# zhouxian/act3d-chained-diffuser

Measured on AMD Instinct MI355X. Metric: train samples/sec (Act3D keypose fwd+bwd+AdamW step), higher is better.
Workload: dtype fp16 / bf16 MFMA on two-part operands (x = hi + lo; fp32 accumulate) in attention; fp32-accurate linears (f32 MFMA; bf16x3 MFMA from 4096 rows); bf16 frozen backbone + FPN; 1 GPU; Act3D keypose training step, 18-PerAct-task shapes: 4 cameras 256x256, 3 ghost-point levels, 1000 ghost points (333/level), E=60, frozen synthetic CLIP-RN50-shaped backbone + trainable FPN included in the step; per_gpu_batch_keyframes=64, global_batch=64, parallelism=dp1, hipgraph=True, backbone_prefetch=True

## Files before the change

### act3d-chained-diffuser_amd/csrc/conv1x1_deep.hip

```cpp
#include "a3d_common.h"
#include "../../include/act3d_hip.h"

namespace a3d {

constexpr int CD_BM = 128, CD_BN = 128, CD_BK = 64;

__device__ __forceinline__ int cd_xoff(int row, int seg) { return row * 64 + ((seg ^ ((row >> 1) & 7)) << 3); }
__device__ __forceinline__ int cd_woff(int row, int seg) { return row * 64 + ((seg ^ ((((row >> 4) & 3) << 1) | ((row >> 1) & 1))) << 3); }

__device__ __forceinline__ unsigned int cd_norm2(unsigned int u, const float* scS, int K, int k, float relu_lo) {
  float a = __uint_as_float(u << 16) * scS[k] + scS[K + k];
  float b = __uint_as_float(u & 0xFFFF0000u) * scS[k + 1] + scS[K + k + 1];
  return pk_bf16(fmaxf(a, relu_lo), fmaxf(b, relu_lo));
}

__device__ __forceinline__ void cd_compute(const unsigned short* Xb, const unsigned short* Wb, const int (&xo)[2][4], const int (&wo)[2][4],
                                           f32x4 (&acc)[4][4]) {
#pragma unroll
  for (int h = 0; h < 2; ++h) {
    s16x8 xa[4], wb[4];
#pragma unroll
    for (int i = 0; i < 4; ++i) {
      xa[i] = *reinterpret_cast<const s16x8*>(&Xb[xo[h][i]]);
      wb[i] = *reinterpret_cast<const s16x8*>(&Wb[wo[h][i]]);
// ... 3 lines not shown
#pragma unroll
      for (int tm = 0; tm < 4; ++tm) acc[tn][tm] = mfma_bf16_16x16x32(wb[tn], xa[tm], acc[tn][tm]);
  }
}

__device__ __forceinline__ void cd_epilogue(f32x4 (&acc)[4][4], float (&ssum)[4][4], float (&ssq)[4][4], unsigned short* __restrict__ y,
                                            long long m0, long long M, int N, int n0, int wm, int wn, int li, int g) {
#pragma unroll
  for (int tm = 0; tm < 4; ++tm) {
    const long long m = m0 + wm * 64 + tm * 16 + li;
    const bool ok = m < M;
    unsigned int pk[8];
#pragma unroll
    for (int tn = 0; tn < 4; ++tn) {
#pragma unroll
      for (int r2 = 0; r2 < 2; ++r2) {
        const unsigned int u = pk_bf16(acc[tn][tm][2 * r2], acc[tn][tm][2 * r2 + 1]);
        const float v0 = ok ? __uint_as_float(u << 16) : 0.f, v1 = ok ? __uint_as_float(u & 0xFFFF0000u) : 0.f;
        ssum[tn][2 * r2] += v0;
        ssq[tn][2 * r2] += v0 * v0;
        ssum[tn][2 * r2 + 1] += v1;
        ssq[tn][2 * r2 + 1] += v1 * v1;
        pk[2 * tn + r2] = u;
      }
      acc[tn][tm] = f32x4{0.f, 0.f, 0.f, 0.f};
    }
    if (ok) {
      uint4* dst = reinterpret_cast<uint4*>(y + (size_t)m * N + n0 + wn * 64 + g * 16);
      dst[0] = make_uint4(pk[0], pk[1], pk[2], pk[3]);
      dst[1] = make_uint4(pk[4], pk[5], pk[6], pk[7]);
    }
  }
}

template <bool XFORM>
__global__ __launch_bounds__(256, 2) void conv1x1_deep_kernel(const unsigned short* __restrict__ x, const unsigned short* __restrict__ w,
                                                            const float* __restrict__ in_scale, const float* __restrict__ in_shift,
                                                            int in_relu, unsigned short* __restrict__ y, float* __restrict__ partial,
                                                            long long M, int N, int K) {
  extern __shared__ __attribute__((aligned(16))) unsigned short smem_cd[];
  unsigned short* Xs = smem_cd;
  unsigned short* Ws = Xs + 2 * CD_BM * CD_BK;
  float* scS = reinterpret_cast<float*>(Ws + 2 * CD_BN * CD_BK);
  const int t = threadIdx.x, lane = t & 63, wave = t >> 6;
  const int li = lane & 15, g = lane >> 4;
  const int wm = wave >> 1, wn = wave & 1;
  const int n0 = blockIdx.y * CD_BN;
  const int KS = K / CD_BK;
  const long long mtiles = (M + CD_BM - 1) / CD_BM;
  if (XFORM)
    for (int i = t; i < K; i += 256) { scS[i] = in_scale[i]; scS[K + i] = in_shift[i]; }
  float ssum[4][4], ssq[4][4];
#pragma unroll
  for (int a = 0; a < 4; ++a)
#pragma unroll
    for (int r = 0; r < 4; ++r) { ssum[a][r] = 0.f; ssq[a][r] = 0.f; }
  const long long my_tiles = blockIdx.x < mtiles ? (mtiles - blockIdx.x + gridDim.x - 1) / gridDim.x : 0;
  const long long total = my_tiles * KS;
  const int srow = t >> 3, sseg = t & 7;
  long long l_m0 = (long long)blockIdx.x * CD_BM;
  int l_ks = 0;
  const float relu_lo = in_relu ? 0.f : -INFINITY;
#define CD_LOAD1(P, i)                                                                                                \
  {                                                                                                                   \
    const long long m_ = l_m0 + srow + 32 * i < M ? l_m0 + srow + 32 * i : M - 1;    \
    P##x##i = *reinterpret_cast<const uint4*>(x + (size_t)m_ * K + l_ks * CD_BK + sseg * 8);                          \
    P##w##i = *reinterpret_cast<const uint4*>(w + (size_t)(n0 + srow + 32 * i) * K + l_ks * CD_BK + sseg * 8);        \
  }
#define CD_LOAD(P)                                                                                                    \
  do {                                                                                                                \
    CD_LOAD1(P, 0) CD_LOAD1(P, 1) CD_LOAD1(P, 2) CD_LOAD1(P, 3)                                                       \
    if (l_left > 1) { --l_left; if (++l_ks == KS) { l_ks = 0; l_m0 += (long long)gridDim.x * CD_BM; } }               \
  } while (0)
#define CD_STAGE1(P, i)                                                                                               \
  {                                                                                                                   \
    uint4 v = P##x##i;                                                                                                \
    if (XFORM) {                                                                                                      \
      const int k0 = ks * CD_BK + sseg * 8;                                                                           \
      unsigned int u0 = v.x, u1 = v.y, u2 = v.z, u3 = v.w;                                                            \
      u0 = cd_norm2(u0, scS, K, k0 + 0, relu_lo); u1 = cd_norm2(u1, scS, K, k0 + 2, relu_lo);                         \
      u2 = cd_norm2(u2, scS, K, k0 + 4, relu_lo); u3 = cd_norm2(u3, scS, K, k0 + 6, relu_lo);                         \
      v = make_uint4(u0, u1, u2, u3);                                                                                 \
    }                                                                                                                 \
    *reinterpret_cast<uint4*>(&Xs[buf * CD_BM * CD_BK + cd_xoff(srow + 32 * i, sseg)]) = v;                           \
    *reinterpret_cast<uint4*>(&Ws[buf * CD_BN * CD_BK + cd_woff(srow + 32 * i, sseg)]) = P##w##i;                     \
  }
#define CD_STAGE(P) CD_STAGE1(P, 0) CD_STAGE1(P, 1) CD_STAGE1(P, 2) CD_STAGE1(P, 3)
  int xo[2][4], wo[2][4];
#pragma unroll
  for (int h = 0; h < 2; ++h)
#pragma unroll
    for (int i = 0; i < 4; ++i) {
      xo[h][i] = cd_xoff(wm * 64 + i * 16 + li, h * 4 + g);
      wo[h][i] = cd_woff(wn * 64 + (li >> 2) * 16 + i * 4 + (li & 3), h * 4 + g);
    }
  if (total > 0) {
    uint4 ax0, ax1, ax2, ax3, aw0, aw1, aw2, aw3, bx0, bx1, bx2, bx3, bw0, bw1, bw2, bw3;
    long long l_left = total;
    CD_LOAD(a);
    CD_LOAD(b);
    long long c_m0 = (long long)blockIdx.x * CD_BM;
    int ks = 0;
    f32x4 acc[4][4];
#pragma unroll
    for (int a = 0; a < 4; ++a)
#pragma unroll
      for (int b = 0; b < 4; ++b) acc[a][b] = f32x4{0.f, 0.f, 0.f, 0.f};
    __syncthreads();
#define CD_STEP(P, BUF)                                                                                               \
    {                                                                                                                 \
      constexpr int buf = BUF;                                                                                        \
      CD_STAGE(P)                                                                                                     \
      CD_LOAD(P);                                                                                \
      __syncthreads();                                             \
      cd_compute(Xs + buf * CD_BM * CD_BK, Ws + buf * CD_BN * CD_BK, xo, wo, acc);                                    \
      if (ks == KS - 1) cd_epilogue(acc, ssum, ssq, y, c_m0, M, N, n0, wm, wn, li, g);                                \
      if (++ks == KS) { ks = 0; c_m0 += (long long)gridDim.x * CD_BM; }                                               \
    }
    for (long long s = 0; s < total; s += 2) {
      CD_STEP(a, 0)
      if (s + 1 < total) CD_STEP(b, 1)
    }
#undef CD_STEP
  }
  if (!partial) return;
  __syncthreads();
  float* redS = reinterpret_cast<float*>(Xs);
  float* redQ = redS + 4 * 64;
#pragma unroll
  for (int tn = 0; tn < 4; ++tn)
#pragma unroll
    for (int r = 0; r < 4; ++r) {
      float sv = ssum[tn][r], q = ssq[tn][r];
#pragma unroll
      for (int o = 1; o < 16; o <<= 1) { sv += __shfl_xor(sv, o, 64); q += __shfl_xor(q, o, 64); }
      if (li == 0) { redS[wave * 64 + g * 16 + tn * 4 + r] = sv; redQ[wave * 64 + g * 16 + tn * 4 + r] = q; }
    }
  __syncthreads();
  if (t < CD_BN) {
    const int wn_i = t >> 6, c = t & 63;
    const float sv = redS[(0 * 2 + wn_i) * 64 + c] + redS[(1 * 2 + wn_i) * 64 + c];
    const float q = redQ[(0 * 2 + wn_i) * 64 + c] + redQ[(1 * 2 + wn_i) * 64 + c];
    float* p = partial + (size_t)blockIdx.x * 2 * N;
    p[n0 + t] = sv;
    p[N + n0 + t] = q;
  }
}

#undef CD_LOAD
#undef CD_LOAD1
#undef CD_STAGE1
#undef CD_STAGE

}

using namespace a3d;

bool a3d::conv1x1_deep_serves(int K, int N) { return K >= 128 && K <= 2048 && (K % CD_BK) == 0 && N >= 128 && N <= 2048 && (N % CD_BN) == 0; }
static size_t cd_lds(int K, bool xform) { return (size_t)2 * (CD_BM + CD_BN) * CD_BK * 2 + (xform ? (size_t)2 * K * sizeof(float) : 0); }

int a3d::conv1x1_deep_slabs(size_t M, int K, int N) {
  (void)K;
  const size_t mtiles = (M + CD_BM - 1) / CD_BM;
  const int nblocks = N / CD_BN;
  return (int)std::min<size_t>(mtiles, (size_t)std::max(1, 512 / nblocks));
}

int a3d::conv1x1_deep_launch(const void* x, const void* w, const float* in_scale, const float* in_shift, int in_relu, void* y, float* partial,
                             size_t M, int K, int N, hipStream_t s) {
  if (in_scale && K > 1024) { set_error("a3d_conv1x1_bn_fwd: the folded BatchNorm-apply of the deep-layer kernel serves K <= 1024 (K=%d)", K); return A3D_ERR_ARG; }
  static bool once = false;
  if (!once) {
    (void)hipFuncSetAttribute((const void*)conv1x1_deep_kernel<false>, hipFuncAttributeMaxDynamicSharedMemorySize, 80 * 1024);
    (void)hipFuncSetAttribute((const void*)conv1x1_deep_kernel<true>, hipFuncAttributeMaxDynamicSharedMemorySize, 80 * 1024);
    once = true;
  }
  const dim3 grid(conv1x1_deep_slabs(M, K, N), N / CD_BN);
  if (in_scale)
    hipLaunchKernelGGL(conv1x1_deep_kernel<true>, grid, dim3(256), cd_lds(K, true), s, (const unsigned short*)x, (const unsigned short*)w,
                       in_scale, in_shift, in_relu, (unsigned short*)y, partial, (long long)M, N, K);
  else
    hipLaunchKernelGGL(conv1x1_deep_kernel<false>, grid, dim3(256), cd_lds(K, false), s, (const unsigned short*)x, (const unsigned short*)w,
                       in_scale, in_shift, in_relu, (unsigned short*)y, partial, (long long)M, N, K);
  return check_launch("a3d_conv1x1_bn_fwd(deep)");
}
```

### act3d-chained-diffuser_amd/lib.py

```python
import ctypes as C
import os

import torch

_PKG_DIR = os.path.dirname(os.path.abspath(__file__))
LIB_PATH = os.path.join(_PKG_DIR, os.path.basename(os.environ.get("A3D_LIB", "libact3d_hip.so")))

_p = C.c_void_p
_i = C.c_int
_f = C.c_float
_d = C.c_double
_z = C.c_size_t
_u64 = C.c_ulonglong



def _struct(name, fields):
    return type(name, (C.Structure,), {"_fields_": [(f, t) for f, t in fields]})


DnHeadParams = _struct("DnHeadParams", [(n, _p) for n in ("enc_w0", "enc_b0", "enc_w1", "enc_b1", "sem", "lang_kv")] +
                       [("S_lang", _i)] + [(n, _p) for n in ("q_w", "q_b", "out_w", "out_b", "ln_g", "ln_b")])
DnCrossParams = _struct("DnCrossParams", [(n, _p) for n in ("sem", "mod", "q_w", "q_b", "freq", "Kf", "Vt")])
DnRestParams = _struct("DnRestParams", [(n, _p) for n in (
    "c_out_w", "c_out_b", "c_ln_g", "c_ln_b", "sem", "s_mod", "s_in_w", "s_in_b", "s_out_w", "s_out_b", "s_ln_g", "s_ln_b", "freq",
    "kmask", "f_mod", "f_w1", "f_b1", "f_w2", "f_b2", "f_ln_g", "f_ln_b")] + [("F", _i)])
DnLayerParams = _struct("DnLayerParams", [("cross", DnCrossParams), ("rest", DnRestParams)])
DnTailParams = _struct("DnTailParams", [(n, _p) for n in (
    "pos_w0", "pos_b0", "pos_w1", "pos_b1", "rot_w0", "rot_b0", "rot_w1", "rot_b1", "noise", "cond_data", "cond_mask", "coef_pos",
    "coef_rot")])

QsParams = _struct("QsParams", [(n, _p) for n in ("wv", "bv", "wo", "bo", "g1", "b1", "w1", "c1", "w2", "c2", "g2", "b2")])
GradReduceRec = _struct("GradReduceRec", [("partial", _p), ("dst", _p), ("bias", _p)] +
                        [(n, _i) for n in ("nsplit", "slab_stride", "count", "row_len", "dst_stride", "group_len")])
QsGrads = _struct("QsGrads", [(n, _p) for n in ("dwv", "dbv", "dwo", "dbo", "dg1", "db1", "dw1", "dc1", "dw2", "dc2", "dg2", "db2")])

SIGNATURES = {
    "a3d_version": (_i, []),
    "a3d_last_error_string": (C.c_char_p, []),
    "a3d_linear_fwd": (_i, [_p, _i, _p, _i, _p, _p, _i, _p, _i, _i, _i, _i, _i, _i, _p]),
    "a3d_linear_wgrad": (_i, [_p, _i, _p, _i, _p, _i, _p, _i, _i, _i, _p]),
    "a3d_linear_wgrad_ws": (_i, [_p, _i, _p, _i, _p, _i, _p, _i, _i, _i, _p, _z, _p]),
    "a3d_linear_wgrad_ws_bytes": (_z, [_i, _i, _i, _i]),
    "a3d_add_layernorm_fwd": (_i, [_p, _p, _p, _p, _p, _p, _p, _i, _i, _f, _p]),
    "a3d_add_layernorm_bwd": (_i, [_p, _p, _p, _p, _p, _p, _p, _p, _p, _i, _i, _p]),
    "a3d_linear_wgrad_partials": (_i, [_p, _i, _p, _i, _i, _i, _i, _i, _p, _z, _p, _p]),
    "a3d_add_layernorm_bwd_partials_count": (_i, [_i, _i]),
    "a3d_add_layernorm_bwd_partials": (_i, [_p, _p, _p, _p, _p, _p, _p, _p, _i, _i, _p]),
    "a3d_colsum_rows_partials": (_i, [_p, _i, _i, _i, _i, _i, _p, _p]),
    "a3d_grad_reduce_table_plan": (_i, [_p, _i, _p]),
    "a3d_grad_reduce_table_upload": (_i, [_p, _p, _i, _p]),
    "a3d_grad_reduce_table": (_i, [_p, _i, _i, _p]),
    "a3d_rope_split_qk": (_i, [_p, _i, _p, _p, _f, _p, _i, _i, _i, _i, _i, _p]),
    "a3d_split_vt": (_i, [_p, _i, _p, _i, _i, _i, _i, _i, _p]),
    "a3d_proj_rope_split": (_i, [_p, _i, _p, _i, _p, _i, _p, _f, _p, _i, _p, _p, _f, _p, _i, _p, _p, _i, _i, _i, _i, _i, _p]),
    "a3d_rope_split": (_i, [_p, _i, _p, _p, _f, _p, _i, _p, _i, _i, _i, _i, _i, _p]),
    "a3d_rope_merge_bwd": (_i, [_p, _i, _p, _p, _f, _p, _i, _i, _i, _i, _i, _i, _p]),
    "a3d_attn_fwd": (_i, [_p, _p, _p, _p, _p, _p, _p, _i, _i, _i, _i, _i, _i, _i, _p]),
    "a3d_attn_fwd_ws_floats": (_z, [_i, _i, _i, _i]),
    "a3d_attn_bwd_bf16": (_i, [_p] * 15 + [_i] * 7 + [_p]),
    "a3d_rope_split16": (_i, [_p, _i, _p, _p, _f, _p, _p, _i, _i, _i, _i, _i, _i, _p]),
    "a3d_proj_rope_split16": (_i, [_p, _i, _p, _i, _p, _i, _p, _f, _p, _p, _i, _p, _f, _p, _p, _i, _p, _i, _i, _i, _i, _i, _p]),
    "a3d_ctx_kv_proj16_splits": (_i, [_i, _i]),
    "a3d_ctx_kv_proj16": (_i, [_p, _i, _p, _p, _p, _p, _p, _p, _p, _p, _p, _i, _p, _i, _i, _i, _i, _i, _i, _i, _p]),
    "a3d_attn16_fwd": (_i, [_p] * 7 + [_i] * 7 + [_p, C.c_uint, _f, _p]),
    "a3d_attn16_fwd_rows": (_i, [_p] * 7 + [_i] * 7 + [_p, C.c_uint, _f, _i, _p]),
    "a3d_conv3x3_tile_count": (_z, [_z, _i, _i]),
    "a3d_conv3x3_dgrad_tiles_ws_ints": (_z, [_z, _i, _i]),
    "a3d_conv3x3_mark_tiles": (_i, [_p, _i, _i, _i, _i, _i, _p, _p]),
    "a3d_conv3x3_dgrad_tiles": (_i, [_p, _p, _p, _p, _p, _z, _i, _i, _p]),
    "a3d_conv3x3_wgrad_tokens_ws_floats": (_z, []),
    "a3d_conv3x3_wgrad_tokens": (_i, [_p, _p, _p, _i, _i, _p, _p, _i, _i, _i, _i, _i, _i, _p]),
    "a3d_attn16_bwd_pack_bytes": (_z, [_i, _i, _i]),
    "a3d_dbg_dn_prof": (_i, [_p]),
    "a3d_attn8_operand_bytes": (_z, [_i, _i, _i]),
    "a3d_attn8_fwd": (_i, [_p] * 8 + [_i] * 7 + [_p]),
    "a3d_attn16_bwd": (_i, [_p] * 16 + [_i] * 7 + [_p, C.c_uint, _f, _p]),
    "a3d_pose_to_signal": (_i, [_p, _p, _p, _i, _i, _p]),
    "a3d_signal_to_pose": (_i, [_p, _p, _p, _i, _i, _p]),
    "a3d_traj_condition": (_i, [_p, _i, _p, _i, _p] + [_p] * 8 + [_i] * 5 + [_p]),
    "a3d_traj_rank": (_i, [_p, _p, _p, _i, _p] + [_f] * 6 + [_p] * 5 + [_i] * 4 + [_p]),
    "a3d_traj_rank_extra": (_i, [_p, _p, _p, _i, _p] + [_f] * 6 + [_p] * 5 + [_i] * 4 + [_p, _f, _p]),
    "a3d_traj_clearance_ws_floats": (_z, [_i] * 5),
    "a3d_traj_clearance": (_i, [_p, _p, _p, _p, _i, _i, _f, _i, _i, _p, _p, _p] + [_i] * 5 + [_p]),
    "a3d_traj_guide_ws_floats": (_z, [_i] * 5),
    "a3d_traj_guide": (_i, [_p, _i, _p, _p, _p, _p, _p, _i, _i, _f, _i, _i, _f, _f, _p, _p] + [_i] * 4 + [_p]),
    "a3d_traj_errors": (_i, [_p, _p, _p, _i, _i, _i, _p]),
    "a3d_keypose_errors": (_i, [_p, _p, _p, _p, _i, _p, _i, _i, _i, _p]),
    "a3d_sym_quat_loss": (_i, [_p, _p, _i, _f, _p, _p, _i, _p]),
    "a3d_sq_fwd_ws_floats": (_z, [_i, _i, _i, _i]),
    "a3d_sq_attn_fwd": (_i, [_p, _p, _p, _i, _p, _p, _i, _p, _p, _p, _p, _p, _p, _p, _i, _i, _i, _i, _i, _p]),
    "a3d_sq_bwd_ws_floats": (_z, [_i, _i, _i, _i]),
    "a3d_sq_attn_bwd": (_i, [_p, _p, _p, _i, _p, _p, _i, _p, _p, _p, _p, _p, _p, _p, _p, _p, _i, _p, _p, _i, _p, _i, _i, _i, _i,
                             _i, _p]),
    "a3d_sq_attn_bwd_acc": (_i, [_p, _p, _p, _i, _p, _p, _i, _p, _p, _p, _p, _p, _p, _p, _p, _p, _i, _p, _p, _i, _p, _i, _i, _i, _i,
                                 _i, _i, _p]),
    "a3d_qs_pre_fwd": (_i, [_p, _p, _p, _p, _p, _f, _p, _i, _i, _i, _p]),
    "a3d_qs_pre_bwd": (_i, [_p, _i, _p, _p, _f, _p, _p, _p, _p, _p, _i, _i, _i, _p]),
    "a3d_qs_save_floats": (_z, [_i, _i]),
    "a3d_qs_post_fwd": (_i, [_p, _p, _p, _p, _p, _i, _i, _i, _p]),
    "a3d_qs_post_bwd": (_i, [_p, _p, _p, _p, _p, _p, _p, _p, _p, _i, _i, _i, _p]),
    "a3d_sq_wgrad_reduce": (_i, [_p, _i, _p, _i, _p, _i, _p]),
    "a3d_dn_head": (_i, [_p, _i, _p, _p, _i, _i, _i, _i, _p]),
    "a3d_dn_cross_ws_floats": (_z, [_i, _i, _i]),
    "a3d_dn_cross": (_i, [_p, _p, _i, _p, _p, _i, _i, _i, _i, _i, _i, _i, _p]),
    "a3d_dn_rest": (_i, [_p, _p, _i, _p, _p, _p, _i, _i, _i, _i, _i, _p]),
    "a3d_dn_tail": (_i, [_p, _p, _p, _i, _p, _p, _i, _i, _i, _i, _p]),
    "a3d_dn_tail_sched": (_i, [_p, _p, _p, _i, _p, _p, _i, _i, _i, _i, _i, _p]),
    "a3d_dn_persist_splits": (_i, [_i, _i]),
    "a3d_dn_persist_sync_ints": (_z, [_i, _i, _i, _i]),
    "a3d_dn_persist_kvx_floats": (_z, [_i, _i, _i]),
    "a3d_dn_persist_prof": (_i, [_p, _i, _i, _i, _i, _p]),
    "a3d_dn_persist_xbuf_floats": (_z, [_i, _i]),
    "a3d_dn_persist": (_i, [_p, _i, _i, _i, _p, _p, _p, _p, _p, _p, _p, _p] + [_i] * 10 + [_p]),
    "a3d_dn_persist_sched": (_i, [_p, _i, _i, _i, _p, _p, _p, _p, _p, _p, _p, _p] + [_i] * 12 + [_p]),
    "a3d_dn_persist_group_of": (_i, [_i, _i, _i, _i, _p]),
    "a3d_dn_persist_group": (_i, [_p, _i, _i, _i, _p, _p, _p, _p, _p, _p, _p, _p] + [_i] * 13 + [_p]),
    "a3d_rope_rows_f32": (_i, [_p, _i, _p, _p, _f, _p, _i, _i, _i, _i, _i, _p]),
    "a3d_dropout": (_i, [_p, _p, _z, _p, C.c_uint, _f, _p]),
    "a3d_dropout_mask": (_i, [_p, _z, _p, C.c_uint, C.c_uint, C.c_uint, _f, _p]),
    "a3d_linear_fwd_drop": (_i, [_p, _i, _p, _i, _p, _p, _i, _p, _i, _i, _i, _i, _i, _i, _p, C.c_uint, _f, _p]),
    "a3d_add_layernorm_bwd_drop": (_i, [_p] * 10 + [_i, _i, _p, C.c_uint, _f, _p]),
    "a3d_attn_fwd_dropout": (_i, [_p, _p, _p, _p, _p, _p, _p, _i, _i, _i, _i, _i, _i, _i, _p, C.c_uint, _f, _p]),
    "a3d_attn_bwd_bf16_dropout": (_i, [_p] * 15 + [_i] * 7 + [_p, C.c_uint, _f, _p]),
    "a3d_pcd_downsample": (_i, [_p, _p, _i, _i, _i, _i, _i, _p]),
    "a3d_knn_topk_ws_bytes": (_z, [_i, _i]),
    "a3d_knn_topk": (_i, [_p, _p, _p, _p, _p, _i, _i, _i, _p]),
    "a3d_traj_nn_topk": (_i, [_p, _i, _p, _p, _p, _p, _i, _i, _i, _p]),
    "a3d_build_context": (_i, [_p, _p, _p, _p, _i, _i, _i, _i, _i, _p]),
    "a3d_build_context_bwd": (_i, [_p, _p, _p, _p, _i, _i, _i, _i, _i, _i, _p]),
    "a3d_build_context_bf16": (_i, [_p, _i, _p, _p, _p, _p, _i, _i, _i, _i, _i, _p]),
    "a3d_colsum_rows_ws_floats": (_z, [_i, _i, _i]),
    "a3d_colsum_rows": (_i, [_p, _i, _i, _i, _i, _i, _p, _i, _p, _p]),
    "a3d_build_context_bwd_bf16": (_i, [_p, _p, _p, _i, _p, _i, _i, _i, _i, _i, _i, _p]),
    "a3d_mask_logits_fwd": (_i, [_p, _p, _p, _i, _i, _i, _p]),
    "a3d_mask_logits_bwd": (_i, [_p, _p, _p, _p, _p, _i, _i, _i, _i, _p]),
    "a3d_argmax_gather": (_i, [_p, _p, _p, _p, _i, _i, _p]),
    "a3d_soft_ce_loss": (_i, [_p, _p, _p, _p, _p, _p, _i, _i, _f, _f, _f, _p]),
    "a3d_elem_loss": (_i, [_p, _p, _i, _i, _f, _p, _p, _p]),
    "a3d_scale_by_scalar": (_i, [_p, _p, _p, _z, _p]),
    "a3d_quat_sigmoid_fwd": (_i, [_p, _p, _p, _i, _p]),
    "a3d_quat_sigmoid_bwd": (_i, [_p, _p, _p, _p, _i, _p]),
    "a3d_ortho6d_sigmoid_fwd": (_i, [_p, _p, _p, _i, _p]),
    "a3d_ortho6d_sigmoid_bwd": (_i, [_p, _p, _p, _p, _i, _p]),
    "a3d_select_row_fwd": (_i, [_p, _p, _p, _i, _i, _i, _p]),
    "a3d_select_row_bwd": (_i, [_p, _p, _p, _i, _i, _i, _p]),
    "a3d_sample_ghost_points": (_i, [_p, _p, _p, _f, _p, _i, _i, _i, _i, _p]),
    "a3d_rng_advance": (_i, [_p, _u64, _p]),
    "a3d_philox4x32_10_host": (None, [_p, _p, _p]),
    "a3d_sincos_host": (None, [_p, _p, _p, _z]),
    "a3d_adamw_step": (_i, [_p, _p, _p, _p, _p, _p, _p, _i, _z, _z, _f, _f, _f, _f, _f, _f, _f, _p]),
    "a3d_adamw_ema_step": (_i, [_p] * 9 + [_i, _z, _z] + [_f] * 9 + [_p]),
    "a3d_adamw_clip_step": (_i, [_p] * 11 + [_i, _z, _z] + [_f] * 10 + [_p]),
    "a3d_adamw_sched_step": (_i, [_p] * 12 + [_i, _z, _z, _i] + [_d] * 3 + [_f] * 9 + [_p]),
    "a3d_swap_f32": (_i, [_p, _p, _z, _p]),
    "a3d_dbg_mfma_bf16": (_i, [_p, _p, _p, _p]),
    "a3d_dbg_mfma_f32": (_i, [_p, _p, _p, _p]),
    "a3d_dbg_cvt_pk_bf16": (_i, [_p, _p, _i, _p]),
    "a3d_bn_nslab": (_i, [_z, _i]),
    "a3d_bn_grid_cap": (_i, [_i]),
    "a3d_conv1x1_streams": (_i, [_i, _i]),
    "a3d_conv1x1_nslab": (_i, [_z, _i, _i]),
    "a3d_conv1x1_bn_fwd": (_i, [_p, _p, _p, _p, _i, _p, _p, _z, _i, _i, _p]),
    "a3d_conv1x1_topdown_serves": (_i, [_i, _i]),
    "a3d_conv1x1_topdown_fwd": (_i, [_p, _p, _p, _i, _p, _p, _z, _i, _i, _i, _i, _p]),
    "a3d_conv1x1_bn_residual_serves": (_i, [_i, _i]),
    "a3d_conv1x1_bn_residual_fwd": (_i, [_p, _p, _p, _p, _i, _p, _p, _p, _p, _p, _i, _i, _p, _z, _i, _i, _p]),
    "a3d_bn_gram_nslab": (_i, [_z, _i]),
    "a3d_bn_gram": (_i, [_p, _p, _p, _i, _p, _p, _z, _i, _i, _p]),
    "a3d_bn_gram_stats": (_i, [_p, _p, _i, _p, _i, _i, _p, _p, _p]),
    "a3d_conv3x3_serves": (_i, [_i, _i, _i, _i]),
    "a3d_conv1x1_deep_mode": (_i, [_i]),
    "a3d_stem_conv_nslab": (_i, [_z, _i, _i]),
    "a3d_stem_conv_bn_fwd": (_i, [_p, _p, _p, _p, _p, _p, _z, _i, _i, _p]),
    "a3d_conv3x3_nslab": (_i, [_z, _i, _i, _i, _i]),
    "a3d_conv3x3_bn_fwd": (_i, [_p, _p, _p, _p, _i, _p, _p, _z, _i, _i, _i, _i, _p]),
    "a3d_bn_stats": (_i, [_p, _p, _z, _i, _i, _p]),
    "a3d_bn_finalize": (_i, [_p, _i, _z, _i, _f, _f, _p, _p, _p, _p, _p, _p, _i, _p]),
    "a3d_bn_apply": (_i, [_p, _p, _p, _p, _p, _p, _p, _z, _i, _i, _p]),
    "a3d_bn_apply_pool2": (_i, [_p, _p, _p, _p, _p, _p, _i, _i, _i, _i, _i, _p]),
    "a3d_rgb_normalize_nhwc_bf16": (_i, [_p, _p, _p, _p, _z, _i, _i, _p]),
    "a3d_upsample2_add_fwd": (_i, [_p, _p, _p, _i, _p, _i, _i, _i, _i, _p]),
    "a3d_upsample2_add_bwd_ws_floats": (_z, [_i, _i, _i, _i]),
    "a3d_upsample2_add_bwd": (_i, [_p, _p, _p, _i, _p, _i, _i, _i, _i, _p]),
    "a3d_ddpm_add_noise": (_i, [_p, _p, _p, _p, _p, _p, _i, _i, _i, _i, _p]),
    "a3d_ddpm_step": (_i, [_p, _p, _p, _p, _p, _p, _p, _p, _i, _i, _i, _i, _p]),
    "a3d_ddpm_step_sched": (_i, [_p, _p, _p, _p, _p, _p, _p, _p, _i, _i, _i, _i, _i, _p]),
    "a3d_adaln_fwd": (_i, [_p, _p, _p, _i, _i, _i, _p]),
    "a3d_adaln_bwd": (_i, [_p, _p, _p, _p, _p, _i, _i, _i, _p]),
    "a3d_sinusoidal_emb": (_i, [_p, _p, _i, _i, _p]),
    "a3d_silu_fwd": (_i, [_p, _p, _z, _p]),
    "a3d_silu_bwd": (_i, [_p, _p, _p, _z, _p]),
    "a3d_add_rows": (_i, [_p, _p, _p, _i, _i, _i, _p]),
    "a3d_add_rows_bwd": (_i, [_p, _p, _i, _i, _i, _p]),
    "a3d_resize_crop": (_i, [_p, _p, _p, _i, _i, _i, _i, _f, _f, _p]),
    "a3d_traj_update": (_i, [_p, _p, _p, _i, _i, _i, _p]),
}

ADAMW_CLIP_WS_DOUBLES = 256
LR_DECAY_KINDS = {"constant": 0, "linear": 1, "cosine": 2}

_lib = None


def load():
    global _lib
    if _lib is not None:
        return _lib
    if not os.path.exists(LIB_PATH):
        raise RuntimeError(
            "libact3d_hip.so is missing (%s). Build it with `python -c 'import __graft_entry__ as g; g.build()'` "
            "(needs hipcc); there is no CPU fallback." % LIB_PATH)
    lib = C.CDLL(LIB_PATH)
    for name, (res, args) in SIGNATURES.items():
        try:
            fn = getattr(lib, name)
        except AttributeError as e:
            raise RuntimeError("libact3d_hip.so does not export %s (stale build?)" % name) from e
        fn.restype = res
        fn.argtypes = args
    _lib = lib
    return lib


def exported_symbols():
    return list(SIGNATURES.keys())


def last_error():
    s = load().a3d_last_error_string()
    return s.decode() if s else ""


def check(rc, what=""):
    if rc != 0:
        raise RuntimeError("libact3d_hip %s failed with code %d: %s" % (what, rc, last_error()))


def ptr(t):
    if t is None:
        return None
    assert t.is_contiguous(), "libact3d_hip needs contiguous tensors"
    return t.data_ptr()


def stream():
    return torch.cuda.current_stream().cuda_stream


def require_gpu(*tensors):
    for t in tensors:
        if t is not None and not t.is_cuda:
            raise RuntimeError("act3d_amd ops run on an MI355X device tensor; got a %s tensor "
                               "(there is no CPU fallback)" % t.device)


def call(name, *args):
    lib = load()
    rc = getattr(lib, name)(*args)
    if rc != 0:
        raise RuntimeError("%s failed with code %d: %s" % (name, rc, last_error()))
```

### include/act3d_hip.h

```cpp
#ifndef ACT3D_HIP_H
#define ACT3D_HIP_H
#include <stddef.h>
#include <stdint.h>
#ifdef __cplusplus
extern "C" {
#endif

int a3d_version(void);
const char* a3d_last_error_string(void);

int a3d_linear_fwd(const float* X, int ldx, const float* W, int ldw, const float* bias, float* Y, int ldy,
                   const float* mask, int ldm, int M, int N, int K, int act, int w_transposed, void* stream);
int a3d_linear_wgrad(const float* dY, int lddy, const float* X, int ldx, float* dW, int lddw, float* db, int M,
                     int N, int K, void* stream);
size_t a3d_linear_wgrad_ws_bytes(int M, int N, int K, int has_bias);
int a3d_linear_wgrad_ws(const float* dY, int lddy, const float* X, int ldx, float* dW, int lddw, float* db, int M,
                        int N, int K, float* ws, size_t ws_bytes, void* stream);
int a3d_add_layernorm_fwd(const float* A, const float* R, const float* gamma, const float* beta, float* Y,
                          float* mean, float* rstd, int M, int E, float eps, void* stream);
int a3d_add_layernorm_bwd(const float* A, const float* R, const float* gamma, const float* mean, const float* rstd,
                          const float* dY, float* dS, float* dgamma, float* dbeta, int M, int E, void* stream);

int a3d_linear_wgrad_partials(const float* dY, int lddy, const float* X, int ldx, int has_bias, int M, int N, int K,
                              float* ws, size_t ws_bytes, int* nsplit_out, void* stream);
// ... 178 lines not shown
                    void* stream);
int a3d_qs_post_bwd(const float* dy, const float* resid, const float* xbar, const float* save, const a3d_qs_params* p,
                    const a3d_qs_grads* gr, float* dxbar, float* cD, float* dresid, int B, int E, int H, void* stream);

int a3d_ddpm_add_noise(const float* x0, const float* noise, const long long* t, const float* acp_pos,
                       const float* acp_rot, float* out, int B, int L, int D, int npos, void* stream);
int a3d_ddpm_step(const float* model_out, const float* sample, const float* noise, const float* cond_data,
                  const unsigned char* cond_mask, const float* coef_pos, const float* coef_rot, float* out, int rows,
                  int D, int npos, int t, void* stream);
int a3d_ddpm_step_sched(const float* model_out, const float* sample, const float* noise, const float* cond_data,
                        const unsigned char* cond_mask, const float* coef_pos, const float* coef_rot, float* out, int rows,
                        int D, int npos, int row, int terminal, void* stream);
int a3d_adaln_fwd(const float* x, const float* mod, float* y, int B, int L, int E, void* stream);
int a3d_adaln_bwd(const float* x, const float* mod, const float* dy, float* dx, float* dmod, int B, int L, int E,
                  void* stream);
int a3d_sinusoidal_emb(const float* x, float* out, int n, int E, void* stream);
int a3d_silu_fwd(const float* x, float* y, size_t n, void* stream);
int a3d_silu_bwd(const float* x, const float* dy, float* dx, size_t n, void* stream);
int a3d_add_rows(const float* x, const float* r, float* y, int B, int L, int E, void* stream);
int a3d_add_rows_bwd(const float* dy, float* dr, int B, int L, int E, void* stream);
int a3d_traj_update(const float* traj, const float* upd, float* out, int rows, int D, int npos, void* stream);

int a3d_pose_to_signal(const float* pose, const float* bounds, float* out, int n, int extra, void* stream);
int a3d_signal_to_pose(const float* signal, const float* bounds, float* out, int n, int extra, void* stream);
int a3d_traj_condition(const float* curr, int ldc, const float* goal, int ldg, const float* bounds, const unsigned char* tmask,
                       const float* init_noise, float* cg, float* gg, float* cond_data, unsigned char* cond_mask,
                       unsigned char* kmask, float* traj, int B, int G, int L, int Dp, int use_goal, void* stream);
int a3d_traj_rank(const float* poses, const unsigned char* tmask, const float* goal, int ldg, const float* bounds,
                  float w_consensus, float w_goal, float w_smooth, float w_length, float w_bounds, float rot_weight, int* best,
                  int* order, float* scores, float* terms, float* selected, int B, int G, int L, int Dp, void* stream);
int a3d_traj_rank_extra(const float* poses, const unsigned char* tmask, const float* goal, int ldg, const float* bounds,
                        float w_consensus, float w_goal, float w_smooth, float w_length, float w_bounds, float rot_weight, int* best,
                        int* order, float* scores, float* terms, float* selected, int B, int G, int L, int Dp, const float* extra,
                        float w_extra, void* stream);
size_t a3d_traj_clearance_ws_floats(int B, int G, int L, int n_points, int n_chunks);
int a3d_traj_clearance(const float* poses, const unsigned char* tmask, const float* scene, const unsigned char* scene_mask, int n_cam,
                       int n_pix, float margin, int skip_head, int skip_tail, float* nearest, float* clearance, float* ws,
                       int n_chunks, int B, int G, int L, int Dp, void* stream);
size_t a3d_traj_guide_ws_floats(int B, int G, int L, int n_points, int n_chunks);
int a3d_traj_guide(float* traj, int D, const unsigned char* tmask, const unsigned char* cond_mask, const float* bounds,
                   const float* scene, const unsigned char* scene_mask, int n_cam, int n_pix, float margin, int skip_head,
                   int skip_tail, float push, float smooth, float* nearest, float* ws, int n_chunks, int B, int G, int L,
                   void* stream);
int a3d_traj_errors(const float* pred, const float* gt, float* cols, int B, int L, int D, void* stream);
int a3d_keypose_errors(const float* pos, const float* rot, const float* grip, const float* gt, int ldgt, float* cols, int B,
                       int nlev, int symmetric, void* stream);
int a3d_sym_quat_loss(const float* q, const float* gt, int ldgt, float coeff, float* loss, float* grad, int B, void* stream);

typedef struct {
  const float *enc_w0, *enc_b0, *enc_w1, *enc_b1;
  const float* sem;
  const float* lang_kv;
  int S_lang;
  const float *q_w, *q_b, *out_w, *out_b, *ln_g, *ln_b;
} a3d_dn_head_params;
typedef struct {
  const float* sem;
  const float* mod;
  const float *q_w, *q_b;
  const float* freq;
  const void* Kf;
  const unsigned short* Vt;
} a3d_dn_cross_params;
typedef struct {
  const float *c_out_w, *c_out_b, *c_ln_g, *c_ln_b;
  const float* sem;
  const float *s_mod, *s_in_w, *s_in_b, *s_out_w, *s_out_b, *s_ln_g, *s_ln_b;
  const float* freq;
  const unsigned char* kmask;
  const float *f_mod, *f_w1, *f_b1, *f_w2, *f_b2, *f_ln_g, *f_ln_b;
  int F;
} a3d_dn_rest_params;
typedef struct {
  const float *pos_w0, *pos_b0, *pos_w1, *pos_b1, *rot_w0, *rot_b0, *rot_w1, *rot_b1;
  const float *noise, *cond_data;
  const unsigned char* cond_mask;
  const float *coef_pos, *coef_rot;
} a3d_dn_tail_params;
int a3d_dn_head(const float* traj, int D, const a3d_dn_head_params* p, float* x_out, int B, int L, int E, int H, void* stream);
size_t a3d_dn_cross_ws_floats(int B, int H, int nsplit);
int a3d_dn_cross(const float* x, const float* traj, int D, const a3d_dn_cross_params* p, float* ws, int B, int L, int E,
                 int H, int S, int Sp, int nsplit, void* stream);
int a3d_dn_rest(const float* x_in, const float* traj, int D, const float* ws, const a3d_dn_rest_params* p, float* x_out,
                int B, int L, int E, int H, int nsplit, void* stream);
int a3d_dn_tail(const float* pos_feats, const float* rot_feats, const float* traj, int D, const a3d_dn_tail_params* p,
                float* traj_out, int B, int L, int E, int t_step, void* stream);
int a3d_dn_tail_sched(const float* pos_feats, const float* rot_feats, const float* traj, int D, const a3d_dn_tail_params* p,
                      float* traj_out, int B, int L, int E, int row, int terminal, void* stream);
typedef struct {
  a3d_dn_cross_params cross;
  a3d_dn_rest_params rest;
} a3d_dn_layer_params;
int a3d_dn_persist_splits(int H, int nsplit);
size_t a3d_dn_persist_kvx_floats(int B, int L, int E);
size_t a3d_dn_persist_xbuf_floats(int B, int L);
int a3d_dn_persist_prof(const int* sync, int B, int L, int n_layers, int nsteps, long long* out256);
size_t a3d_dn_persist_sync_ints(int B, int L, int n_layers, int nsteps);
int a3d_dn_persist(const a3d_dn_layer_params* layers_dev, int n_traj, int n_pos, int n_rot, const a3d_dn_head_params* head,
                   const a3d_dn_tail_params* tail, float* traj, float* qbuf, float* part, float* kvx, float* xbuf, int* sync, int B,
                   int L, int D, int E, int H, int S, int Sp, int nsplit, int t_first, int nsteps, void* stream);
int a3d_dn_persist_sched(const a3d_dn_layer_params* layers_dev, int n_traj, int n_pos, int n_rot, const a3d_dn_head_params* head,
                         const a3d_dn_tail_params* tail, float* traj, float* qbuf, float* part, float* kvx, float* xbuf, int* sync,
                         int B, int L, int D, int E, int H, int S, int Sp, int nsplit, int row_first, int nsteps, int n_rows,
                         int last_terminal, void* stream);
int a3d_dn_persist_group_of(int B, int L, int n_cand, int traj, int* out5);
int a3d_dn_persist_group(const a3d_dn_layer_params* layers_dev, int n_traj, int n_pos, int n_rot, const a3d_dn_head_params* head,
                         const a3d_dn_tail_params* tail, float* traj, float* qbuf, float* part, float* kvx, float* xbuf, int* sync,
                         int B, int L, int D, int E, int H, int S, int Sp, int nsplit, int row_first, int nsteps, int n_rows,
                         int last_terminal, int n_cand, void* stream);
int a3d_dbg_dn_prof(long long* out18);
int a3d_rope_rows_f32(const float* Y, int ldy, const float* xyz, const float* freq, float scale, float* out, int B, int N,
                      int Npad, int E, int H, void* stream);

int a3d_bn_nslab(size_t rows, int C);
int a3d_bn_stats(const void* x, float* partial , size_t rows, int C, int nslab, void* stream);
int a3d_bn_finalize(const float* partial, int nslab, size_t rows, int C, float eps, float momentum, const float* gamma,
                    const float* beta, float* running_mean, float* running_var, float* scale, float* shift, int train,
                    void* stream);
int a3d_bn_apply(const void* x, const void* residual, const float* res_scale, const float* res_shift, const float* scale,
                 const float* shift, void* y, size_t rows, int C, int relu, void* stream);
int a3d_bn_apply_pool2(const void* x, const void* residual, const float* scale, const float* shift, void* y_full,
                       void* y_pool, int N, int H, int W, int C, int relu, void* stream);
int a3d_bn_grid_cap(int cap);
int a3d_upsample2_add_fwd(const void* lat, const void* top, const float* bias, int nbias, void* y, int N, int H, int W, int C,
                          void* stream);
size_t a3d_upsample2_add_bwd_ws_floats(int N, int H, int W, int C);
int a3d_upsample2_add_bwd(const void* dy, void* dtop, float* dbias, int nbias, float* ws, int N, int H, int W, int C,
                          void* stream);

int a3d_rgb_normalize_nhwc_bf16(const float* x, const float* mean, const float* stdv, void* y, size_t N, int H, int W,
                                void* stream);

int a3d_dbg_mfma_bf16(const void* A16x32, const void* B32x16, float* D16x16, void* stream);
int a3d_dbg_mfma_f32(const float* A16x4, const float* B4x16, float* D16x16, void* stream);
int a3d_dbg_cvt_pk_bf16(const float* in, void* out, int npairs, void* stream);

int a3d_conv1x1_streams(int K, int N);
int a3d_conv1x1_nslab(size_t M, int K, int N);
int a3d_conv1x1_bn_fwd(const void* x, const void* w, const float* in_scale, const float* in_shift, int in_relu, void* y,
                       float* partial, size_t M, int K, int N, void* stream);
int a3d_conv1x1_topdown_serves(int K, int N);
int a3d_conv1x1_topdown_fwd(const void* x, const void* w, const float* bias, int nbias, const void* top, void* y, size_t images,
                            int H, int W, int K, int N, void* stream);
int a3d_conv1x1_bn_residual_serves(int K, int N);
int a3d_conv1x1_bn_residual_fwd(const void* x, const void* w, const float* in_scale, const float* in_shift, int in_relu,
                                const float* out_scale, const float* out_shift, const void* res, const float* res_scale,
                                const float* res_shift, int relu, int round_conv, void* y, size_t M, int K, int N, void* stream);
int a3d_bn_gram_nslab(size_t M, int K);
int a3d_bn_gram(const void* x, const float* in_scale, const float* in_shift, int in_relu, float* gpart, float* spart, size_t M, int K,
                int nslab, void* stream);
int a3d_bn_gram_stats(const float* gpart, const float* spart, int nslab, const void* w, int K, int N, double* work, float* stats,
                      void* stream);
int a3d_conv1x1_deep_mode(int mode);
int a3d_stem_conv_nslab(size_t images, int H, int W);
int a3d_stem_conv_bn_fwd(const float* rgb, const float* mean, const float* stdv, const void* w, void* y, float* partial, size_t images,
                         int H, int W, void* stream);

int a3d_conv3x3_serves(int Cin, int Cout, int H, int W);
int a3d_conv3x3_nslab(size_t images, int H, int W, int Cin, int Cout);
int a3d_conv3x3_bn_fwd(const void* x, const void* w, const float* in_scale, const float* in_shift, int in_relu, void* y,
                       float* partial, size_t images, int H, int W, int Cin, int Cout, void* stream);

int a3d_resize_crop(const float* src, float* dst, const int* params, int frames, int planes, int H, int W, float scale,
                    float shift, void* stream);

#ifdef __cplusplus
}
#endif
#endif
```

Measured before the change: 3749 samples/s.

## Add 256x128 eight-wave variant of the deep conv1x1 kernel and enable by default

Adds a new deep 1x1 conv kernel that uses eight waves (4x2) per block with 256x128 output tiles, so each weight tile is reused across more rows. It keeps the register-prefetched double-buffered LDS pipeline, packs the BN scale and shift into float4 for a paired FMA, and splits the MFMA compute around staging. The grid is halved to match, and partial BN stats are written per 128-row slab. The goal is more reuse and latency hiding per block, at the cost of more LDS per block (up to 112KB), which may reduce occupancy. An environment or API switch selects it, defaulting to the new variant, and a probe script is added to benchmark the variants.

```diff
diff --git a/act3d-chained-diffuser_amd/csrc/conv1x1_deep.hip b/act3d-chained-diffuser_amd/csrc/conv1x1_deep.hip
--- a/act3d-chained-diffuser_amd/csrc/conv1x1_deep.hip
+++ b/act3d-chained-diffuser_amd/csrc/conv1x1_deep.hip
@@ -179,12 +179,212 @@
 #undef CD_STAGE1
 #undef CD_STAGE
 
+
+typedef float f32x2 __attribute__((ext_vector_type(2)));
+
+__device__ __forceinline__ unsigned int cd_norm2p(unsigned int u, float4 p, float relu_lo) {
+  f32x2 v = {__uint_as_float(u << 16), __uint_as_float(u & 0xFFFF0000u)};
+  v = __builtin_elementwise_fma(v, f32x2{p.x, p.y}, f32x2{p.z, p.w});
+  return pk_bf16(fmaxf(v.x, relu_lo), fmaxf(v.y, relu_lo));
+}
+
+__device__ __forceinline__ void cd_compute_half(const unsigned short* Xb, const unsigned short* Wb, int xo, int wo, f32x4 (&acc)[4][4]) {
+  s16x8 xa[4], wb[4];
+#pragma unroll
+  for (int i = 0; i < 4; ++i) {
+    xa[i] = *reinterpret_cast<const s16x8*>(&Xb[xo + i * 16 * CD_BK]);
+    wb[i] = *reinterpret_cast<const s16x8*>(&Wb[wo + i * 4 * CD_BK]);
+  }
+#pragma unroll
+  for (int tn = 0; tn < 4; ++tn)
+#pragma unroll
+    for (int tm = 0; tm < 4; ++tm) acc[tn][tm] = mfma_bf16_16x16x32(wb[tn], xa[tm], acc[tn][tm]);
+}
+
+template <bool RAGGED>
+__device__ __forceinline__ void cd_epilogue1(f32x4 (&acc)[4][4], f32x2 (&ssum)[4][2], f32x2 (&ssq)[4][2], unsigned short* __restrict__ y,
+                                             long long mw, long long M, int N, int col, int li) {
+#pragma unroll
+  for (int tm = 0; tm < 4; ++tm) {
+    const long long m = mw + tm * 16 + li;
+    const bool ok = !RAGGED || m < M;
+    unsigned int pk[8];
+#pragma unroll
+    for (int tn = 0; tn < 4; ++tn) {
+#pragma unroll
+      for (int r2 = 0; r2 < 2; ++r2) {
+        const unsigned int u = pk_bf16(acc[tn][tm][2 * r2], acc[tn][tm][2 * r2 + 1]);
+        f32x2 v = {__uint_as_float(u << 16), __uint_as_float(u & 0xFFFF0000u)};
+        if (RAGGED && !ok) v = f32x2{0.f, 0.f};
+        ssum[tn][r2] += v;
+        ssq[tn][r2] = __builtin_elementwise_fma(v, v, ssq[tn][r2]);
+        pk[2 * tn + r2] = u;
+      }
+      acc[tn][tm] = f32x4{0.f, 0.f, 0.f, 0.f};
+    }
+    if (ok) {
+      uint4* dst = reinterpret_cast<uint4*>(y + (size_t)m * N + col);
+      dst[0] = make_uint4(pk[0], pk[1], pk[2], pk[3]);
+      dst[1] = make_uint4(pk[4], pk[5], pk[6], pk[7]);
+    }
+  }
+}
+
+constexpr int CD1_WM = 4, CD1_WN = 2;
+template <bool XFORM>
+__global__ __launch_bounds__(64 * CD1_WM * CD1_WN, 2) void conv1x1_deep_kernel_v1(const unsigned short* __restrict__ x, const unsigned short* __restrict__ w,
+                                                                          const float* __restrict__ in_scale, const float* __restrict__ in_shift,
+                                                                          int in_relu, unsigned short* __restrict__ y, float* __restrict__ partial,
+                                                                          long long M, int N, int K) {
+  constexpr int WM = CD1_WM, WN = CD1_WN, BM = 64 * WM, BN = 64 * WN, NT = 64 * WM * WN;
+  constexpr int RS = NT / 8;
+  constexpr int NX = BM / RS, NW = BN / RS;
+  static_assert(NX <= 4 && NW <= 4 && NX >= 1 && NW >= 1, "register sets hold up to four pieces per operand");
+  extern __shared__ __attribute__((aligned(16))) unsigned short smem_cd[];
+  unsigned short* Xs = smem_cd;
+  unsigned short* Ws = Xs + 2 * BM * CD_BK;
+  float4* scS = reinterpret_cast<float4*>(Ws + 2 * BN * CD_BK);
+  const int t = threadIdx.x, lane = t & 63, wave = t >> 6;
+  const int li = lane & 15, g = lane >> 4;
+  const int wm = wave / WN, wn = wave % WN;
+  const int n0 = blockIdx.y * BN;
+  const int KS = K / CD_BK;
+  const long long mtiles = (M + BM - 1) / BM;
+  if (XFORM)
+    for (int i = t; i < K / 2; i += NT) scS[i] = make_float4(in_scale[2 * i], in_scale[2 * i + 1], in_shift[2 * i], in_shift[2 * i + 1]);
+  f32x2 ssum[4][2], ssq[4][2];
+#pragma unroll
+  for (int a = 0; a < 4; ++a)
+#pragma unroll
+    for (int r = 0; r < 2; ++r) { ssum[a][r] = f32x2{0.f, 0.f}; ssq[a][r] = f32x2{0.f, 0.f}; }
+  const long long my_tiles = blockIdx.x < mtiles ? (mtiles - blockIdx.x + gridDim.x - 1) / gridDim.x : 0;
+  const long long total = my_tiles * KS;
+  const int srow = t >> 3, sseg = t & 7;
+  const float relu_lo = in_relu ? 0.f : -INFINITY;
+  long long l_m0 = (long long)blockIdx.x * BM;
+  int l_ks = 0;
+  const unsigned short *xp0, *xp1, *xp2, *xp3;
+  const unsigned short* const wp = w + (size_t)(n0 + srow) * K + sseg * 8;
+#define CD_XPTR(i) xp##i = x + (size_t)(l_m0 + srow + RS * i < M ? l_m0 + srow + RS * i : M - 1) * K + sseg * 8;
+#define CD_XPTRS CD_XPTR(0) CD_XPTR(1) CD_XPTR(2) CD_XPTR(3)
+  CD_XPTRS
+#define CD_LOAD1(P, i)                                                                                                \
+  {                                                                                                                   \
+    if (i < NX) P##x##i = *reinterpret_cast<const uint4*>(xp##i + l_ks * CD_BK);                                      \
+    if (i < NW) P##w##i = *reinterpret_cast<const uint4*>(wp + (size_t)(RS * i) * K + l_ks * CD_BK);                  \
+  }
+#define CD_LOAD(P)                                                                                                    \
+  do {                                                                                                                \
+    CD_LOAD1(P, 0) CD_LOAD1(P, 1) CD_LOAD1(P, 2) CD_LOAD1(P, 3)                                                       \
+    if (l_left > 1) { --l_left; if (++l_ks == KS) { l_ks = 0; l_m0 += (long long)gridDim.x * BM; CD_XPTRS } }         \
+  } while (0)
+#define CD_STAGE1(P, i)                                                                                               \
+  {                                                                                                                   \
+    if (i < NX) {                                                                                                     \
+      uint4 v = P##x##i;                                                                                              \
+      if (XFORM) v = make_uint4(cd_norm2p(v.x, p0, relu_lo), cd_norm2p(v.y, p1, relu_lo), cd_norm2p(v.z, p2, relu_lo), cd_norm2p(v.w, p3, relu_lo)); \
+      *reinterpret_cast<uint4*>(&Xs[buf * BM * CD_BK + cd_xoff(srow + RS * i, sseg)]) = v;                            \
+    }                                                                                                                 \
+    if (i < NW) *reinterpret_cast<uint4*>(&Ws[buf * BN * CD_BK + cd_woff(srow + RS * i, sseg)]) = P##w##i;            \
+  }
+#define CD_STAGE(P)                                                                                                   \
+  {                                                                                                                   \
+    float4 p0, p1, p2, p3;                                                                                            \
+    if (XFORM) { const float4* pp = scS + kst * (CD_BK / 2) + sseg * 4; p0 = pp[0]; p1 = pp[1]; p2 = pp[2]; p3 = pp[3]; } \
+    CD_STAGE1(P, 0) CD_STAGE1(P, 1) CD_STAGE1(P, 2) CD_STAGE1(P, 3)                                                   \
+  }
+  int xo[2], wo[2];
+#pragma unroll
+  for (int h = 0; h < 2; ++h) {
+    xo[h] = cd_xoff(wm * 64 + li, h * 4 + g);
+    wo[h] = cd_woff(wn * 64 + (li >> 2) * 16 + (li & 3), h * 4 + g);
+  }
+  if (total > 0) {
+    uint4 ax0, ax1, ax2, ax3, aw0, aw1, aw2, aw3, bx0, bx1, bx2, bx3, bw0, bw1, bw2, bw3;
+    long long l_left = total;
+    CD_LOAD(a);
+    CD_LOAD(b);
+    long long c_m0 = (long long)blockIdx.x * BM;
+    int ks = 0;
+    f32x4 acc[4][4];
+#pragma unroll
+    for (int a = 0; a < 4; ++a)
+#pragma unroll
+      for (int b = 0; b < 4; ++b) acc[a][b] = f32x4{0.f, 0.f, 0.f, 0.f};
+    __syncthreads();
+    { constexpr int buf = 0; const int kst = 0; CD_STAGE(a) }
+    CD_LOAD(a);
+#define CD_STEP(P, BUF)                                                                                               \
+    {                                                                                                                 \
+      __syncthreads();                                             \
+      cd_compute_half(Xs + BUF * BM * CD_BK, Ws + BUF * BN * CD_BK, xo[0], wo[0], acc);                               \
+      {                                                                                                               \
+        constexpr int buf = 1 - BUF;                                                                                  \
+        const int kst = ks + 1 == KS ? 0 : ks + 1;                                                                    \
+        CD_STAGE(P)                                                                                                   \
+        CD_LOAD(P);                                                                                   \
+      }                                                                                                               \
+      cd_compute_half(Xs + BUF * BM * CD_BK, Ws + BUF * BN * CD_BK, xo[1], wo[1], acc);                               \
+      if (ks == KS - 1) {                                                                                             \
+        const long long mw = c_m0 + wm * 64;                                                                          \
+        if (c_m0 + BM <= M) cd_epilogue1<false>(acc, ssum, ssq, y, mw, M, N, n0 + wn * 64 + g * 16, li);              \
+        else cd_epilogue1<true>(acc, ssum, ssq, y, mw, M, N, n0 + wn * 64 + g * 16, li);                              \
+      }                                                                                                               \
+      if (++ks == KS) { ks = 0; c_m0 += (long long)gridDim.x * BM; }                                                  \
+    }
+    for (long long s = 0; s + 1 < total; s += 2) {
+      CD_STEP(b, 0)
+      CD_STEP(a, 1)
+    }
+    if (total & 1) CD_STEP(b, 0)
+#undef CD_STEP
+  }
+  if (!partial) return;
+  __syncthreads();
+  float* redS = reinterpret_cast<float*>(Xs);
+  float* redQ = redS + WM * WN * 64;
+#pragma unroll
+  for (int tn = 0; tn < 4; ++tn)
+#pragma unroll
+    for (int r = 0; r < 4; ++r) {
+      float sv = ssum[tn][r >> 1][r & 1], q = ssq[tn][r >> 1][r & 1];
+#pragma unroll
+      for (int o = 1; o < 16; o <<= 1) { sv += __shfl_xor(sv, o, 64); q += __shfl_xor(q, o, 64); }
+      if (li == 0) { redS[wave * 64 + g * 16 + tn * 4 + r] = sv; redQ[wave * 64 + g * 16 + tn * 4 + r] = q; }
+    }
+  __syncthreads();
+  if (t < BN * (WM / 2)) {
+    const int half = t / BN, c = t % BN, wn_i = c >> 6, cc = c & 63;
+    const int w0 = (2 * half) * WN + wn_i, w1 = (2 * half + 1) * WN + wn_i;
+    const long long slab = (long long)blockIdx.x * (WM / 2) + half;
+    if (slab * 128 < M) {
+      float* p = partial + (size_t)slab * 2 * N;
+      p[n0 + c] = redS[w0 * 64 + cc] + redS[w1 * 64 + cc];
+      p[N + n0 + c] = redQ[w0 * 64 + cc] + redQ[w1 * 64 + cc];
+    }
+  }
+}
+
+#undef CD_LOAD
+#undef CD_LOAD1
+#undef CD_STAGE1
+#undef CD_STAGE
+#undef CD_XPTR
+#undef CD_XPTRS
+
 }
 
 using namespace a3d;
 
 bool a3d::conv1x1_deep_serves(int K, int N) { return K >= 128 && K <= 2048 && (K % CD_BK) == 0 && N >= 128 && N <= 2048 && (N % CD_BN) == 0; }
 static size_t cd_lds(int K, bool xform) { return (size_t)2 * (CD_BM + CD_BN) * CD_BK * 2 + (xform ? (size_t)2 * K * sizeof(float) : 0); }
+
+static int cd_variant = getenv("A3D_CONV1X1_DEEP_VARIANT") ? (atoi(getenv("A3D_CONV1X1_DEEP_VARIANT")) > 0 ? 1 : 0) : 1;
+extern "C" int a3d_conv1x1_deep_variant(int variant) {
+  const int prev = cd_variant;
+  if (variant >= 0) cd_variant = variant > 0 ? 1 : 0;
+  return prev;
+}
 
 int a3d::conv1x1_deep_slabs(size_t M, int K, int N) {
   (void)K;
@@ -193,9 +393,26 @@
   return (int)std::min<size_t>(mtiles, (size_t)std::max(1, 512 / nblocks));
 }
 
+template <bool XFORM>
+static void cd_launch_v1(const void* x, const void* w, const float* in_scale, const float* in_shift, int in_relu, void* y, float* partial,
+                         size_t M, int K, int N, hipStream_t s) {
+  static bool once = false;
+  if (!once) { (void)hipFuncSetAttribute((const void*)conv1x1_deep_kernel_v1<XFORM>, hipFuncAttributeMaxDynamicSharedMemorySize, 112 * 1024); once = true; }
+  const int slabs = conv1x1_deep_slabs(M, K, N);
+  const dim3 grid((slabs + 1) / 2, N / (64 * CD1_WN));
+  const size_t lds = (size_t)2 * 64 * (CD1_WM + CD1_WN) * CD_BK * 2 + (XFORM ? (size_t)2 * K * sizeof(float) : 0);
+  hipLaunchKernelGGL(conv1x1_deep_kernel_v1<XFORM>, grid, dim3(64 * CD1_WM * CD1_WN), lds, s, (const unsigned short*)x, (const unsigned short*)w,
+                     in_scale, in_shift, in_relu, (unsigned short*)y, partial, (long long)M, N, K);
+}
+
 int a3d::conv1x1_deep_launch(const void* x, const void* w, const float* in_scale, const float* in_shift, int in_relu, void* y, float* partial,
                              size_t M, int K, int N, hipStream_t s) {
   if (in_scale && K > 1024) { set_error("a3d_conv1x1_bn_fwd: the folded BatchNorm-apply of the deep-layer kernel serves K <= 1024 (K=%d)", K); return A3D_ERR_ARG; }
+  if (cd_variant != 0) {
+    if (in_scale) cd_launch_v1<true>(x, w, in_scale, in_shift, in_relu, y, partial, M, K, N, s);
+    else cd_launch_v1<false>(x, w, in_scale, in_shift, in_relu, y, partial, M, K, N, s);
+    return check_launch("a3d_conv1x1_bn_fwd(deep)");
+  }
   static bool once = false;
   if (!once) {
     (void)hipFuncSetAttribute((const void*)conv1x1_deep_kernel<false>, hipFuncAttributeMaxDynamicSharedMemorySize, 80 * 1024);
diff --git a/act3d-chained-diffuser_amd/lib.py b/act3d-chained-diffuser_amd/lib.py
--- a/act3d-chained-diffuser_amd/lib.py
+++ b/act3d-chained-diffuser_amd/lib.py
@@ -171,6 +171,7 @@
     "a3d_bn_gram_stats": (_i, [_p, _p, _i, _p, _i, _i, _p, _p, _p]),
     "a3d_conv3x3_serves": (_i, [_i, _i, _i, _i]),
     "a3d_conv1x1_deep_mode": (_i, [_i]),
+    "a3d_conv1x1_deep_variant": (_i, [_i]),
     "a3d_stem_conv_nslab": (_i, [_z, _i, _i]),
     "a3d_stem_conv_bn_fwd": (_i, [_p, _p, _p, _p, _p, _p, _z, _i, _i, _p]),
     "a3d_conv3x3_nslab": (_i, [_z, _i, _i, _i, _i]),
diff --git a/include/act3d_hip.h b/include/act3d_hip.h
--- a/include/act3d_hip.h
+++ b/include/act3d_hip.h
@@ -354,6 +354,7 @@
 int a3d_bn_gram_stats(const float* gpart, const float* spart, int nslab, const void* w, int K, int N, double* work, float* stats,
                       void* stream);
 int a3d_conv1x1_deep_mode(int mode);
+int a3d_conv1x1_deep_variant(int variant);
 int a3d_stem_conv_nslab(size_t images, int H, int W);
 int a3d_stem_conv_bn_fwd(const float* rgb, const float* mean, const float* stdv, const void* w, void* y, float* partial, size_t images,
                          int H, int W, void* stream);
diff --git a/profiles/conv1x1_deep_variants_probe.py b/profiles/conv1x1_deep_variants_probe.py
--- /dev/null
+++ b/profiles/conv1x1_deep_variants_probe.py
@@ -0,0 +1,102 @@
+import argparse
+import importlib
+import json
+import os
+import statistics
+import sys
+
+import torch
+import torch.nn.functional as F
+
+sys.path.insert(0, os.path.dirname(os.path.dirname(os.path.abspath(__file__))))
+a3d = importlib.import_module("act3d-chained-diffuser_amd")
+L = a3d.lib
+lib = L.load()
+dev = torch.device("cuda:0")
+
+ap = argparse.ArgumentParser()
+ap.add_argument("--images", type=int, default=256)
+ap.add_argument("--rounds", type=int, default=5)
+ap.add_argument("--iters", type=int, default=10)
+ap.add_argument("--variants", default="")
+ap.add_argument("--counters", action="store_true")
+ap.add_argument("--out", default="")
+args = ap.parse_args()
+
+SHAPES = [(256, 1024, 16, 6), (512, 2048, 8, 3), (1024, 256, 16, 5), (1024, 2048, 8, 1), (512, 1024, 16, 1), (1024, 512, 16, 1),
+          (512, 256, 32, 1), (256, 512, 32, 1), (512, 128, 32, 3), (2048, 512, 8, 2)]
+has_switch = hasattr(lib, "a3d_conv1x1_deep_variant")
+variants = [int(v) for v in args.variants.split(",")] if args.variants else ([0, 1] if has_switch else [0])
+torch.backends.cudnn.benchmark = True
+
+
+def window(fn, iters):
+    a, b = torch.cuda.Event(enable_timing=True), torch.cuda.Event(enable_timing=True)
+    a.record()
+    for _ in range(iters):
+        fn()
+    b.record()
+    torch.cuda.synchronize()
+    return a.elapsed_time(b) / iters * 1e3
+
+
+rows = []
+prev = lib.a3d_conv1x1_deep_variant(-1) if has_switch else 0
+try:
+    for K, N, hw, count in SHAPES:
+        M = args.images * hw * hw
+        g = torch.Generator(device="cpu").manual_seed(K * 7 + N)
+        x = torch.randn(M, K, generator=g).to(dev).to(torch.bfloat16)
+        w = (torch.randn(N, K, generator=g) / K ** 0.5).to(dev).to(torch.bfloat16)
+        sc = (torch.rand(2, K, generator=g) + 0.5).to(dev)
+        y = torch.empty(M, N, device=dev, dtype=torch.bfloat16)
+        part = torch.empty(max(1, lib.a3d_conv1x1_nslab(M, K, N)), 2, N, device=dev)
+        x4 = x.view(args.images, hw, hw, K).permute(0, 3, 1, 2)
+        w4 = w.view(N, K, 1, 1).contiguous(memory_format=torch.channels_last)
+        st = L.stream()
+
+        def ours(v, xform):
+            def fn():
+                if has_switch:
+                    lib.a3d_conv1x1_deep_variant(v)
+                L.call("a3d_conv1x1_bn_fwd", x.data_ptr(), w.data_ptr(), sc[0].data_ptr() if xform else None,
+                       sc[1].data_ptr() if xform else None, 1 if xform else 0, y.data_ptr(), part.data_ptr(), M, K, N, st)
+            return fn
+
+        arms = {}
+        for v in variants:
+            arms["v%d_plain" % v] = ours(v, False)
+            if K <= 1024:
+                arms["v%d_apply" % v] = ours(v, True)
+        if args.counters:
+            for fn in arms.values():
+                fn()
+            torch.cuda.synchronize()
+            continue
+        arms["library_gemm"] = lambda: F.conv2d(x4, w4)
+        for fn in arms.values():
+            for _ in range(3):
+                fn()
+        torch.cuda.synchronize()
+        t = {k: [] for k in arms}
+        for _ in range(args.rounds):
+            for k, fn in arms.items():
+                t[k].append(window(fn, args.iters))
+        row = {"K": K, "N": N, "hw": hw, "launches": count, "M": M, "out_MB": round(2.0 * M * N / 1e6, 1), "in_MB": round(2.0 * M * K / 1e6, 1)}
+        for k, v in t.items():
+            row[k + "_us"] = round(statistics.median(v), 1)
+            row[k + "_min_us"] = round(min(v), 1)
+        rows.append(row)
+        print(row, flush=True)
+finally:
+    if has_switch:
+        lib.a3d_conv1x1_deep_variant(prev)
+if not args.counters:
+    res = {"images": args.images, "rounds": args.rounds, "iters": args.iters, "variants": variants, "shapes": rows,
+           "step_us": {k[:-3]: round(sum(r[k] * r["launches"] for r in rows if k in r), 1)
+                       for k in rows[0] if k.endswith("_us") and not k.endswith("_min_us") and all(k in r for r in rows)}}
+    print(json.dumps(res))
+    if args.out:
+        os.makedirs(os.path.dirname(os.path.abspath(args.out)), exist_ok=True)
+        with open(args.out, "w") as f:
+            json.dump(res, f, indent=1)
```

Measured after the change: 3744 samples/s. No clear change (-0.1%).
